# gabrevaya/LatentDiffEq.jl

Measured on NVIDIA B200. Metric: latent trajectory-steps/sec (forward solve + gradient, the reference's ForwardDiffSensitivity semantics), higher is better.
Workload: dtype f32

## Files before the change

### latentdiffeq.jl_b200/csrc/ldeq_api.cu

```cuda
#include <cmath>
#include <cstdio>
#include <cstdlib>
#include <cstring>

#include "ldeq_internal.h"
#include "ldeq_rhs.cuh"
#include "ldeq_tsit5.cuh"
#include "ldeq_julia_trig.cuh"

namespace ldeq {

cudaError_t launch_erk_fwd(int solver, int dtype, bool friction, bool with_tape, const void* z0, const void* theta, const double* tg, int B,
                           int T, const KOpts& ko, void* traj, int32_t* ret, int32_t* na, int32_t* nr, const TapeView<float>& tv,
                           const GridInfo& gi, cudaStream_t s);

int set_err(ldeq_handle* h, int code, const char* what, cudaError_t ce) {
    if (h) {
        h->err = what ? what : "";
        if (ce != cudaSuccess) {
            h->err += ": ";
            h->err += cudaGetErrorString(ce);
        }
    }
    return code;
// ... 152 lines not shown
    if (tape) tv = fwd_tape_view<float>(tape, theta, tg);
    KOpts kov = ko;
    GridInfo giv = gi;
    void* args[] = {&z0, &theta, &tg, &B, &T, &kov, &traj, &ret, &na, &nr, &tv, &giv};
    const int grid = (B + LDEQ_FWD_THREADS - 1) / LDEQ_FWD_THREADS;
    const size_t es = dtype == LDEQ_F32 ? 4 : 8;
    void* kfn = fn[(dtype == LDEQ_F32 ? 0 : 2) + (tape ? 1 : 0)];
    return cudaLaunchKernel(kfn, dim3(grid), dim3(LDEQ_FWD_THREADS), args, ring_smem(rhs->z_dim, es, LDEQ_FWD_THREADS, T), s);
}
static cudaError_t launch_user_bwd(void* const* fn, const ldeq_tape* tape, const void* dtraj, int ld, void* dz0, void* dtheta, cudaStream_t s) {
    TapeView<float> tv{tape->t, (float*)tape->u, tape->info, tape->cap, nullptr, nullptr, nullptr, nullptr, nullptr};
    const void* theta = tape->theta;
    const double* tg = tape->tgrid;
    int B = tape->B, T = tape->T;
    const int32_t* ret = tape->retcode;
    const int32_t* na = tape->naccept;
    GridInfo giv{tape->grid_t0, tape->grid_h, tape->grid_uniform, ld, bwd_sort_lanes()};
    void* args[] = {&theta, &tg, &B, &T, &dtraj, &tv, &ret, &na, &dz0, &dtheta, &giv};
    const int grid = (B + LDEQ_BWD_THREADS - 1) / LDEQ_BWD_THREADS;
    const size_t es = tape->dtype == LDEQ_F32 ? 4 : 8;
    void* kfn = fn[tape->dtype == LDEQ_F32 ? 4 : 5];
    return cudaLaunchKernel(kfn, dim3(grid), dim3(LDEQ_BWD_THREADS), args, ring_smem(tape->z_dim, es, LDEQ_BWD_THREADS, T), s);
}

static cudaError_t launch_user_fwdsens(void* const* fn, const ldeq_tape* tape, const void* dtraj, int ld, void* dz0, void* dtheta, cudaStream_t s) {
    const void* z0 = tape->u;
    const void* theta = tape->theta;
    const double* tg = tape->tgrid;
    int B = tape->B, T = tape->T, np = 1;
    GridInfo gi{tape->grid_t0, tape->grid_h, tape->grid_uniform, ld};
    KOpts kov = tape->kopts;
    const int32_t* ret = tape->retcode;
    const int32_t* key = tape->naccept;
    const int grid = (B + 127) / 128;
    const int base = tape->dtype == LDEQ_F32 ? 6 : 8;
    void* args_p[] = {&z0, &theta, &tg, &B, &gi, &T, &kov, &np, &key, &dtraj, &ret, &dtheta};
    cudaError_t e = cudaLaunchKernel(fn[base], dim3(grid), dim3(128), args_p, 0, s);
    if (e != cudaSuccess) return e;
    void* args_u[] = {&z0, &theta, &tg, &B, &gi, &T, &kov, &np, &key, &dtraj, &ret, &dz0};
    return cudaLaunchKernel(fn[base + 1], dim3(grid), dim3(128), args_u, 0, s);
}

bool slot_acquire(ldeq_handle* h, int32_t** h_info, cudaEvent_t* ev) {
    for (const ldeq_handle::Slot& sl : h->deferred_slots) slot_release(h, sl.h_info, sl.ev);
    h->deferred_slots.clear();
    if (h->free_slots.empty()) {
        const int n = 64;
        int32_t* blk = nullptr;
        if (cudaMallocHost((void**)&blk, n * 2 * sizeof(int32_t)) != cudaSuccess) return false;
        h->pinned_blocks.push_back(blk);
        for (int i = 0; i < n; ++i) {
            cudaEvent_t e;
            if (cudaEventCreateWithFlags(&e, cudaEventDisableTiming) != cudaSuccess) return false;
            h->free_slots.push_back({blk + 2 * i, e});
        }
    }
    ldeq_handle::Slot sl = h->free_slots.back();
    h->free_slots.pop_back();
    *h_info = sl.h_info;
    *ev = sl.ev;
    return true;
}
void slot_release(ldeq_handle* h, int32_t* h_info, cudaEvent_t ev) {
    if (h_info && ev) {
        cudaEventSynchronize(ev);
        if (h) h->free_slots.push_back({h_info, ev});
    }
}
static bool slot_get(ldeq_handle* h, ldeq_tape* tape) { return slot_acquire(h, &tape->h_info, &tape->ready); }
static void slot_put(ldeq_handle* h, ldeq_tape* tape, cudaStream_t s) {
    if (tape->ready && capturing(s))
        h->deferred_slots.push_back({tape->h_info, tape->ready});
    else
// ... 596 lines not shown
```

### latentdiffeq.jl_b200/csrc/ldeq_erk_fwdsens.cu

```cuda
#include "ldeq_fwdsens_kernels.cuh"

namespace ldeq {

template <class MD, class S, bool FR>
static cudaError_t launch_t(const ldeq_tape* tp, const void* dtraj, int ld, void* dz0, void* dtheta, cudaStream_t s) {
    const int B = tp->B, grid = (B + LDEQ_FWDSENS_THREADS - 1) / LDEQ_FWDSENS_THREADS;
    const GridInfo gi{tp->grid_t0, tp->grid_h, tp->grid_uniform, ld};
    const int* key = fwdsens_sort_key(tp);
    erk_fwdsens_kernel<MD, S, 1, FR, true><<<grid, LDEQ_FWDSENS_THREADS, 0, s>>>((const S*)tp->u, (const S*)tp->theta, tp->tgrid, B, gi, tp->T, tp->kopts,
                                                                                1, key, (const S*)dtraj, tp->retcode, (S*)dtheta);
    erk_fwdsens_kernel<MD, S, 2, FR, false><<<grid, LDEQ_FWDSENS_THREADS, 0, s>>>((const S*)tp->u, (const S*)tp->theta, tp->tgrid, B, gi, tp->T, tp->kopts,
                                                                                 1, key, (const S*)dtraj, tp->retcode, (S*)dz0);
    return cudaGetLastError();
}

template <class MD>
static cudaError_t launch_m(const ldeq_tape* tp, const void* dtraj, int ld, void* dz0, void* dtheta, cudaStream_t s) {
    const bool fr = tp->rhs_kind == LDEQ_RHS_PENDULUM_FRICTION;
    if (tp->dtype == LDEQ_F32)
        return fr ? launch_t<MD, float, true>(tp, dtraj, ld, dz0, dtheta, s) : launch_t<MD, float, false>(tp, dtraj, ld, dz0, dtheta, s);
    return fr ? launch_t<MD, double, true>(tp, dtraj, ld, dz0, dtheta, s) : launch_t<MD, double, false>(tp, dtraj, ld, dz0, dtheta, s);
}

cudaError_t launch_erk_fwdsens(const ldeq_tape* tp, const void* dtraj, int ld, void* dz0, void* dtheta, cudaStream_t s) {
    switch (tp->solver) {
        case LDEQ_SOLVER_DP5: return launch_m<ErkDual<TabDP5>>(tp, dtraj, ld, dz0, dtheta, s);
        case LDEQ_SOLVER_BS3: return launch_m<ErkDual<TabBS3>>(tp, dtraj, ld, dz0, dtheta, s);
        case LDEQ_SOLVER_RK4: return launch_m<ErkDual<TabRK4>>(tp, dtraj, ld, dz0, dtheta, s);
        default: return cudaErrorInvalidValue;
    }
}

}
```

### latentdiffeq.jl_b200/csrc/ldeq_fwdsens.cu

```cuda
#include "ldeq_fwdsens_kernels.cuh"

namespace ldeq {

template <class S, bool FR>
static cudaError_t launch_fwdsens_t(const ldeq_tape* tp, const void* dtraj, int ld, void* dz0, void* dtheta, cudaStream_t s) {
    const int B = tp->B, grid = (B + LDEQ_FWDSENS_THREADS - 1) / LDEQ_FWDSENS_THREADS;
    const GridInfo gi{tp->grid_t0, tp->grid_h, tp->grid_uniform, ld};
    const int* key = fwdsens_sort_key(tp);
    tsit5_fwdsens_kernel<S, 1, FR, true><<<grid, LDEQ_FWDSENS_THREADS, 0, s>>>((const S*)tp->u, (const S*)tp->theta, tp->tgrid, B, gi, tp->T, tp->kopts, 1, key,
                                                             (const S*)dtraj, tp->retcode, (S*)dtheta);
    tsit5_fwdsens_kernel<S, 2, FR, false><<<grid, LDEQ_FWDSENS_THREADS, 0, s>>>((const S*)tp->u, (const S*)tp->theta, tp->tgrid, B, gi, tp->T, tp->kopts, 1, key,
                                                              (const S*)dtraj, tp->retcode, (S*)dz0);
    return cudaGetLastError();
}

cudaError_t launch_fwdsens(const ldeq_tape* tp, const void* dtraj, int ld, void* dz0, void* dtheta, cudaStream_t s) {
    if (tp->solver != LDEQ_SOLVER_TSIT5) return launch_erk_fwdsens(tp, dtraj, ld, dz0, dtheta, s);
    const bool fr = tp->rhs_kind == LDEQ_RHS_PENDULUM_FRICTION;
    if (tp->dtype == LDEQ_F32)
        return fr ? launch_fwdsens_t<float, true>(tp, dtraj, ld, dz0, dtheta, s) : launch_fwdsens_t<float, false>(tp, dtraj, ld, dz0, dtheta, s);
    return fr ? launch_fwdsens_t<double, true>(tp, dtraj, ld, dz0, dtheta, s) : launch_fwdsens_t<double, false>(tp, dtraj, ld, dz0, dtheta, s);
}

}
```

### latentdiffeq.jl_b200/csrc/ldeq_fwdsens.cuh

```cuda
#pragma once

#include "ldeq_dual.cuh"
#include "ldeq_erk.cuh"

namespace ldeq {

#define LDEQ_DL _Pragma("unroll") for (int i_ = 0; i_ < N; ++i_)
template <class S, int N> __device__ __forceinline__ Dual<S, N> dual_fma(S s, Dual<S, N> k, Dual<S, N> acc) {
    acc.v = s_fma<S>(s, k.v, acc.v);
    LDEQ_DL acc.d[i_] = s_fma<S>(s, k.d[i_], acc.d[i_]);
    return acc;
}
template <class S, int N> __device__ __forceinline__ Dual<S, N> dual_scale(S a, Dual<S, N> b) {
    b.v *= a;
    LDEQ_DL b.d[i_] *= a;
    return b;
}
template <class S, int N> __device__ __forceinline__ Dual<S, N> dual_axpy_time(Dual<S, N> uprev, double dt, Dual<S, N> sum) {
    Dual<S, N> r;
    r.v = (S)fma(dt, (double)sum.v, (double)uprev.v);
    LDEQ_DL r.d[i_] = (S)fma(dt, (double)sum.d[i_], (double)uprev.d[i_]);
    return r;
}
template <class S, int N> __device__ __forceinline__ Dual<S, N> dual_scale_time(double dt, Dual<S, N> sum) {
    Dual<S, N> r;
    r.v = (S)(dt * (double)sum.v);
    LDEQ_DL r.d[i_] = (S)(dt * (double)sum.d[i_]);
    return r;
}
template <class S, int N> __device__ __forceinline__ S dual_sse(Dual<S, N> a, bool wp) {
    S s = a.v * a.v;
    if (wp) { LDEQ_DL s += a.d[i_] * a.d[i_]; }
    return s;
}
template <class S, int N> __device__ __forceinline__ S dual_absnorm(Dual<S, N> a, bool wp) { return wp ? s_sqrt<S>(dual_sse(a, true)) : s_abs<S>(a.v); }
template <class S, int N> __device__ __forceinline__ Dual<S, N> dual_div_s(Dual<S, N> a, S s) {
    a.v /= s;
    LDEQ_DL a.d[i_] /= s;
    return a;
}
template <class S, int N> __device__ __forceinline__ S dual_rms(const Dual<S, N>* a, int n, bool wp) {
    S s = (S)0;
    for (int i = 0; i < n; ++i) s += dual_sse(a[i], wp);
    const int len = wp ? n * (1 + N) : n;
    return s_sqrt<S>(s / (S)len);
}
#undef LDEQ_DL

#ifndef LDEQ_FWDSENS_PREFETCH_ROWS
#define LDEQ_FWDSENS_PREFETCH_ROWS 24
#endif
#ifndef LDEQ_FWDSENS_THREADS
#define LDEQ_FWDSENS_THREADS 128
#endif

__device__ __forceinline__ void prefetch_l1(const void* p) { asm volatile("prefetch.global.L1 [%0];" ::"l"(p)); }

struct Tsit5Dual {
    static constexpr int NS = 7, ORDER = 5;
    template <class RHS, class S, int NP>
    __device__ __forceinline__ static void step(const Dual<S, NP>* u, const Dual<S, NP>* L, double t, double dts,
                                                Dual<S, NP> (*k)[RHS::ZD], Dual<S, NP>* unew) {
        constexpr int Z = RHS::ZD;
        using D = Dual<S, NP>;
        using Tb = Tab<S>;
        D tmp[Z], sum;
        for (int i = 0; i < Z; ++i) { sum = dual_scale(Tb::a21, k[0][i]); tmp[i] = dual_axpy_time(u[i], dts, sum); }
        RHS::f(k[1], tmp, L, t + Tb::c2 * dts);
        for (int i = 0; i < Z; ++i) {
            sum = dual_scale(Tb::a31, k[0][i]); sum = dual_fma(Tb::a32, k[1][i], sum);
            tmp[i] = dual_axpy_time(u[i], dts, sum);
        }
        RHS::f(k[2], tmp, L, t + Tb::c3 * dts);
        for (int i = 0; i < Z; ++i) {
            sum = dual_scale(Tb::a41, k[0][i]); sum = dual_fma(Tb::a42, k[1][i], sum); sum = dual_fma(Tb::a43, k[2][i], sum);
            tmp[i] = dual_axpy_time(u[i], dts, sum);
        }
        RHS::f(k[3], tmp, L, t + Tb::c4 * dts);
        for (int i = 0; i < Z; ++i) {
            sum = dual_scale(Tb::a51, k[0][i]); sum = dual_fma(Tb::a52, k[1][i], sum); sum = dual_fma(Tb::a53, k[2][i], sum);
            sum = dual_fma(Tb::a54, k[3][i], sum);
            tmp[i] = dual_axpy_time(u[i], dts, sum);
        }
        RHS::f(k[4], tmp, L, t + Tb::c5 * dts);
        for (int i = 0; i < Z; ++i) {
            sum = dual_scale(Tb::a61, k[0][i]); sum = dual_fma(Tb::a62, k[1][i], sum); sum = dual_fma(Tb::a63, k[2][i], sum);
            sum = dual_fma(Tb::a64, k[3][i], sum); sum = dual_fma(Tb::a65, k[4][i], sum);
            tmp[i] = dual_axpy_time(u[i], dts, sum);
        }
        RHS::f(k[5], tmp, L, t + dts);
        for (int i = 0; i < Z; ++i) {
            sum = dual_scale(Tb::a71, k[0][i]); sum = dual_fma(Tb::a72, k[1][i], sum); sum = dual_fma(Tb::a73, k[2][i], sum);
            sum = dual_fma(Tb::a74, k[3][i], sum); sum = dual_fma(Tb::a75, k[4][i], sum); sum = dual_fma(Tb::a76, k[5][i], sum);
            unew[i] = dual_axpy_time(u[i], dts, sum);
        }
        RHS::f(k[6], unew, L, t + dts);
    }
    template <class S, int NP, int Z>
    __device__ __forceinline__ static Dual<S, NP> err_sum(Dual<S, NP> (*k)[Z], int i) {
        using Tb = Tab<S>;
        Dual<S, NP> sum = dual_scale(Tb::bt1, k[0][i]);
        sum = dual_fma(Tb::bt2, k[1][i], sum); sum = dual_fma(Tb::bt3, k[2][i], sum);
        sum = dual_fma(Tb::bt4, k[3][i], sum); sum = dual_fma(Tb::bt5, k[4][i], sum); sum = dual_fma(Tb::bt6, k[5][i], sum);
        sum = dual_fma(Tb::bt7, k[6][i], sum);
        return sum;
    }
    __device__ __forceinline__ static void dense_c(const double* kk, double* c2, double* c3, double* c4) {
        using Td = Tab<double>;
        *c2 = fma(Td::r72, kk[6], fma(Td::r62, kk[5], fma(Td::r52, kk[4], fma(Td::r42, kk[3], fma(Td::r32, kk[2], fma(Td::r22, kk[1], Td::r12 * kk[0]))))));
        *c3 = fma(Td::r73, kk[6], fma(Td::r63, kk[5], fma(Td::r53, kk[4], fma(Td::r43, kk[3], fma(Td::r33, kk[2], fma(Td::r23, kk[1], Td::r13 * kk[0]))))));
        *c4 = fma(Td::r74, kk[6], fma(Td::r64, kk[5], fma(Td::r54, kk[4], fma(Td::r44, kk[3], fma(Td::r34, kk[2], fma(Td::r24, kk[1], Td::r14 * kk[0]))))));
    }
};

template <class TB> struct ErkDual {
    static constexpr int NS = TB::NS, ORDER = TB::ORDER;
    template <class RHS, class S, int NP>
    __device__ __forceinline__ static void step(const Dual<S, NP>* u, const Dual<S, NP>* L, double t, double dts,
                                                Dual<S, NP> (*k)[RHS::ZD], Dual<S, NP>* unew) {
        constexpr int Z = RHS::ZD;
        using D = Dual<S, NP>;
        D tmp[Z];
#pragma unroll
        for (int j = 1; j < NS; ++j) {
            for (int i = 0; i < Z; ++i) {
                D sum = D((S)0);
                bool first = true;
#pragma unroll
                for (int l = 0; l < j; ++l) {
                    if (TB::a(j, l) == 0.0) continue;
                    sum = first ? dual_scale((S)TB::a(j, l), k[l][i]) : dual_fma((S)TB::a(j, l), k[l][i], sum);
                    first = false;
                }
                if (j < NS - 1) tmp[i] = dual_axpy_time(u[i], dts, sum);
                else unew[i] = dual_axpy_time(u[i], dts, sum);
            }
            if (j < NS - 1) RHS::f(k[j], tmp, L, t + TB::c(j) * dts);
            else RHS::f(k[j], unew, L, t + dts);
        }
    }
    template <class S, int NP, int Z>
    __device__ __forceinline__ static Dual<S, NP> err_sum(Dual<S, NP> (*k)[Z], int i) {
        Dual<S, NP> sum = Dual<S, NP>((S)0);
        bool first = true;
#pragma unroll
        for (int j = 0; j < NS; ++j) {
            if (TB::bt(j) == 0.0) continue;
            sum = first ? dual_scale((S)TB::bt(j), k[j][i]) : dual_fma((S)TB::bt(j), k[j][i], sum);
            first = false;
        }
        return sum;
    }
    __device__ __forceinline__ static void dense_c(const double* kk, double* c2, double* c3, double* c4) {
        double c[3] = {0.0, 0.0, 0.0};
#pragma unroll
        for (int m = 1; m < 4; ++m)
#pragma unroll
            for (int j = 0; j < NS; ++j)
                if (erk_r<TB>(j, m) != 0.0) c[m - 1] = fma(erk_r<TB>(j, m), kk[j], c[m - 1]);
        *c2 = c[0]; *c3 = c[1]; *c4 = c[2];
    }
};

template <class M, class RHS, class S, int NP, bool SEED_P>
__device__ __forceinline__ void
erk_fwdsens_body(const S* __restrict__ z0, const S* __restrict__ theta, const double* __restrict__ tg, int B, GridInfo gi, int T,
                   KOpts o, int norm_partials, const int* __restrict__ sort_key, const S* __restrict__ dtraj, const int* __restrict__ primal_ret,
                   S* __restrict__ dout) {
    constexpr int Z = RHS::ZD, PD = RHS::PD;
    using D = Dual<S, NP>;
    constexpr int NS = M::NS;
    int b = blockIdx.x * blockDim.x + threadIdx.x;
    const int ld = gi.ld;
    auto tgrid = [&](int k) -> double { return gi.uniform ? fma((double)k, gi.h, gi.t0) : tg[k]; };
    const bool wp = norm_partials != 0;
    if (sort_key) {
        __shared__ int s_key[LDEQ_FWDSENS_THREADS];
        __shared__ short s_order[LDEQ_FWDSENS_THREADS];
        const int tid = threadIdx.x, nt = blockDim.x;
        const int key = b < B ? sort_key[b] : 0x7fffffff;
        s_key[tid] = key;
        __syncthreads();
        int rank = 0;
        for (int j = 0; j < nt; ++j) {
            const int kj = s_key[j];
            rank += (kj < key || (kj == key && j < tid)) ? 1 : 0;
        }
        s_order[rank] = (short)tid;
        __syncthreads();
        b = blockIdx.x * blockDim.x + s_order[tid];
    }
    if (b >= B) return;
    D u[Z], k[NS][Z], unew[Z], tmp[Z], sum, L[PD + RHS::NPRE];
    const double t0 = tg[0], tend = tg[T - 1];
    const double dtmax = o.dtmax > 0.0 ? o.dtmax : (tend - t0);
    const double dtmin = o.dtmin > 0.0 ? o.dtmin : fmax(2.220446049250313e-16, ulp_of(t0));
    const S abstol = (S)o.abstol, reltol = (S)o.reltol;
    double acc[NP];
    double t = t0, dt = o.dt;
    {
        {
            for (int i = 0; i < Z; ++i) {
                u[i] = D(z0[(size_t)b * Z + i]);
                if (!SEED_P) u[i].d[i] = (S)1;
            }
            for (int i = 0; i < PD; ++i) {
                L[i] = D(theta[(size_t)b * PD + i]);
                if (SEED_P) L[i].d[i] = (S)1;
            }
            RHS::prepare(L);
            RHS::f(k[0], u, L, t0);
            if (o.adaptive && !(o.dt > 0.0)) {
                S sk[Z];
                for (int i = 0; i < Z; ++i) {
                    sk[i] = abstol + dual_absnorm(u[i], wp) * reltol;
                    tmp[i] = dual_div_s(u[i], sk[i]);
                }
                const double d0 = (double)dual_rms(tmp, Z, wp);
                for (int i = 0; i < Z; ++i) tmp[i] = dual_div_s(k[0][i], sk[i]);
                const double d1 = (double)dual_rms(tmp, Z, wp);
                double dt0 = (d0 < 1e-5 || d1 < 1e-5) ? 1e-6 : 0.01 * (d0 / d1);
                dt0 = fmin(dt0, dtmax);
                if (dt0 < 10.0 * 2.220446049250313e-16) {
                    dt = fmax(1e-6, dtmin);
                } else {
                    D u1[Z], f1[Z];
                    for (int i = 0; i < Z; ++i) u1[i] = dual_axpy_time(u[i], dt0, k[0][i]);
                    RHS::f(f1, u1, L, t0 + dt0);
                    for (int i = 0; i < Z; ++i) tmp[i] = dual_div_s(f1[i] - k[0][i], sk[i]);
                    const double d2 = (double)dual_rms(tmp, Z, wp) / dt0;
                    const double m = fmax(d1, d2);
                    const double dt1 = (m <= 1e-15) ? fmax(1e-6, dt0 * 1e-3) : ::pow(10.0, -(2.0 + log10(m)) / (double)M::ORDER);
                    dt = fmax(dtmin, fmin(100.0 * dt0, fmin(dt1, dtmax)));
                }
            }
        }
    }
#pragma unroll
    for (int q = 0; q < NP; ++q) acc[q] = 0.0;
    for (int i = 0; i < Z; ++i)
#pragma unroll
        for (int q = 0; q < NP; ++q) acc[q] += (double)u[i].d[q] * (double)dtraj[(size_t)b * Z + i];
    PiState pst = pi_init(o);
    int ks = 1, ret = RET_SUCCESS;
    long long iters = 0;
    if (!(dt > 0.0) || !isfinite(dt)) ret = RET_DTLESSTHANMIN;
    int kpf = 1;
    S dvn[Z];
#pragma unroll
    for (int i = 0; i < Z; ++i) dvn[i] = T > 1 ? dtraj[((size_t)ld + b) * Z + i] : (S)0;
    while (ks < T && ret == RET_SUCCESS) {
        if (iters >= o.maxiters) { ret = RET_MAXITERS; break; }
        ++iters;
        {
            const int hi = ks + LDEQ_FWDSENS_PREFETCH_ROWS < T ? ks + LDEQ_FWDSENS_PREFETCH_ROWS : T;
            for (; kpf < hi; ++kpf) prefetch_l1(dtraj + ((size_t)kpf * ld + b) * Z);
        }
        const double dts = fmin(dt, tend - t);
        double tnew = t + dts;
        if (::fabs(tnew - tend) < 100.0 * ulp_of(fmax(::fabs(t), ::fabs(tend)))) tnew = tend;
        M::template step<RHS, S, NP>(u, L, t, dts, k, unew);
        double EEst = 0.0;
// ... 26 lines not shown
                for (int i = 0; i < Z; ++i) dv[i] = dvn[i];
                if (ks + 1 < T) {
#pragma unroll
                    for (int i = 0; i < Z; ++i) dvn[i] = dtraj[((size_t)(ks + 1) * ld + b) * Z + i];
                }
                if (tsv == tnew) {
#pragma unroll
                    for (int i = 0; i < Z; ++i)
#pragma unroll
                        for (int q = 0; q < NP; ++q) acc[q] += (double)unew[i].d[q] * (double)dv[i];
                } else {
                    const S th = (S)((tsv - t) * inv);
                    const S a1 = (S)dts * th, a2 = a1 * th, a3 = a2 * th, a4 = a3 * th;
#pragma unroll
                    for (int i = 0; i < Z; ++i) {
                        wsum[i] += dv[i];
                        w1[i] = s_fma<S>(a1, dv[i], w1[i]);
                        w2[i] = s_fma<S>(a2, dv[i], w2[i]);
                        w3[i] = s_fma<S>(a3, dv[i], w3[i]);
                        w4[i] = s_fma<S>(a4, dv[i], w4[i]);
                    }
                    interior = true;
                }
                ++ks;
                tsv = ks < T ? tgrid(ks) : 0.0;
            }
            if (interior) {
#pragma unroll
                for (int i = 0; i < Z; ++i)
#pragma unroll
                    for (int q = 0; q < NP; ++q) {
                        double kk[NS], c2, c3, c4;
#pragma unroll
                        for (int j = 0; j < NS; ++j) kk[j] = (double)k[j][i].d[q];
                        const double k1 = kk[0];
                        M::dense_c(kk, &c2, &c3, &c4);
                        acc[q] += (double)u[i].d[q] * (double)wsum[i] +
                                  (k1 * (double)w1[i] + c2 * (double)w2[i] + c3 * (double)w3[i] + c4 * (double)w4[i]);
                    }
            }
            t = tnew;
            for (int i = 0; i < Z; ++i) { u[i] = unew[i]; k[0][i] = k[NS - 1][i]; }
        }
        if (o.adaptive) dt = dt_next;
        if (ks < T && o.adaptive && (!(::fabs(dt) > dtmin) || !isfinite(dt))) { ret = RET_DTLESSTHANMIN; break; }
    }
    const bool ok = ret == RET_SUCCESS && primal_ret[b] == RET_SUCCESS;
#pragma unroll
    for (int q = 0; q < NP; ++q) dout[(size_t)b * NP + q] = ok ? (S)acc[q] : (S)0;
}

template <class RHS, class S, int NP, bool SEED_P>
__device__ __forceinline__ void
tsit5_fwdsens_body(const S* __restrict__ z0, const S* __restrict__ theta, const double* __restrict__ tg, int B, GridInfo gi, int T,
                   KOpts o, int norm_partials, const int* __restrict__ sort_key, const S* __restrict__ dtraj, const int* __restrict__ primal_ret,
                   S* __restrict__ dout) {
    erk_fwdsens_body<Tsit5Dual, RHS, S, NP, SEED_P>(z0, theta, tg, B, gi, T, o, norm_partials, sort_key, dtraj, primal_ret, dout);
}

}
```

### latentdiffeq.jl_b200/csrc/ldeq_fwdsens_kernels.cuh

```cuda
#pragma once
#include "ldeq_internal.h"
#include "ldeq_fwdsens.cuh"
#include <cstdlib>

#ifndef LDEQ_FWDSENS_MINBLOCKS
#define LDEQ_FWDSENS_MINBLOCKS 5
#endif

namespace ldeq {

template <bool FRICTION> struct PendulumDualRHS {
    static constexpr int ZD = 2, PD = 1;
    static constexpr int NPRE = 1;
    template <class D> __device__ __forceinline__ static void prepare(D* p) {
        typedef typename D::value_type S;
        const D G((S)10.0f);
        p[PD] = -G / p[0];
    }
    template <class D> __device__ __forceinline__ static void f(D* du, const D* u, const D* p, double) {
        typedef typename D::value_type S;
        du[0] = u[1];
        const D a = p[PD] * sin(u[0]);
        if (FRICTION) {
            const S bm = (S)0.7f / (S)1.0f;
            du[1] = a - bm * u[1];
        } else {
            du[1] = a;
        }
    }
};

template <class S, int NP, bool FRICTION, bool SEED_P>
__global__ void __launch_bounds__(LDEQ_FWDSENS_THREADS, LDEQ_FWDSENS_MINBLOCKS)
tsit5_fwdsens_kernel(const S* __restrict__ z0, const S* __restrict__ theta, const double* __restrict__ tg, int B, GridInfo gi, int T,
                     KOpts o, int norm_partials, const int* __restrict__ sort_key, const S* __restrict__ dtraj, const int* __restrict__ primal_ret,
                     S* __restrict__ dout) {
    tsit5_fwdsens_body<PendulumDualRHS<FRICTION>, S, NP, SEED_P>(z0, theta, tg, B, gi, T, o, norm_partials, sort_key, dtraj, primal_ret, dout);
}

template <class MD, class S, int NP, bool FRICTION, bool SEED_P>
__global__ void __launch_bounds__(LDEQ_FWDSENS_THREADS, LDEQ_FWDSENS_MINBLOCKS)
erk_fwdsens_kernel(const S* __restrict__ z0, const S* __restrict__ theta, const double* __restrict__ tg, int B, GridInfo gi, int T,
                   KOpts o, int norm_partials, const int* __restrict__ sort_key, const S* __restrict__ dtraj, const int* __restrict__ primal_ret,
                   S* __restrict__ dout) {
    erk_fwdsens_body<MD, PendulumDualRHS<FRICTION>, S, NP, SEED_P>(z0, theta, tg, B, gi, T, o, norm_partials, sort_key, dtraj, primal_ret, dout);
}

inline const int* fwdsens_sort_key(const ldeq_tape* tp) {
    static const bool sort = [] { const char* e = getenv("LDEQ_FWDSENS_SORT"); return !(e && e[0] == '0'); }();
    return sort ? tp->naccept : nullptr;
}

}
```

### latentdiffeq.jl_b200/csrc/ldeq_internal.h

```cpp
#pragma once

#include <cuda_runtime.h>
#include <stdint.h>

#include <string>
#include <vector>

#include "../../include/ldeq.h"
#include "ldeq_common.cuh"

#define LDEQ_MAX_SLABS 8
#define LDEQ_GRID_CACHE 16

struct ldeq_handle {
    int device = 0;
    std::string err;
    int64_t launches = 0;
    double* d_tgrid = nullptr;
    size_t d_tgrid_cap = 0;
    std::vector<double> h_tgrid;
    double grid_t0 = 0.0, grid_h = 0.0;
    int grid_uniform = 0;
    struct GridEntry {
        std::vector<double> t;
// ... 41 lines not shown
    const ldeq_rhs* rhs = nullptr;
    void* base = nullptr;
    double* t = nullptr;
    void* u = nullptr;
    void* theta = nullptr;
    double* tgrid = nullptr;
    int32_t* retcode = nullptr;
    int32_t* naccept = nullptr;
    int32_t* nreject = nullptr;
    int32_t* info = nullptr;
    int32_t* h_info = nullptr;
    cudaEvent_t ready = nullptr;
    bool checked = false;
    ldeq::KOpts kopts;
    double grid_t0 = 0.0, grid_h = 0.0;
    int grid_uniform = 0;
    int sense = 0;
    int solver = 0;
    std::vector<ldeq_tape*> parts;
    std::vector<int> part_b0;
};

namespace ldeq {

int set_err(ldeq_handle* h, int code, const char* what, cudaError_t ce = cudaSuccess);
bool capturing(cudaStream_t s);
int refuse_capture(ldeq_handle* h, cudaStream_t s, const char* what, const char* why);
int upload_tgrid(ldeq_handle* h, const double* t_host, int T, cudaStream_t s);
int ensure_scratch(ldeq_handle* h, int slot, size_t bytes, cudaStream_t s);
KOpts to_kopts(const ldeq_opts* o);
int bwd_sort_lanes();
bool slot_acquire(ldeq_handle* h, int32_t** h_info, cudaEvent_t* ev);
void slot_release(ldeq_handle* h, int32_t* h_info, cudaEvent_t ev);
cudaError_t launch_fwdsens(const ldeq_tape* tape, const void* dtraj, int ld, void* dz0, void* dtheta, cudaStream_t s);
cudaError_t launch_erk_fwdsens(const ldeq_tape* tape, const void* dtraj, int ld, void* dz0, void* dtheta, cudaStream_t s);
cudaError_t launch_erk_bwd(const ldeq_tape* tape, const void* dtraj, int ld, void* dz0, void* dtheta, cudaStream_t s);
void* const* user_rhs_kernels(ldeq_handle* h, const ldeq_rhs* rhs, int solver);

#define LDEQ_CUDA(call)                                                    \
    do {                                                                   \
        cudaError_t _e = (call);                                           \
        if (_e != cudaSuccess) return ldeq::set_err(h, LDEQ_ERR_CUDA, #call, _e); \
    } while (0)

}
```

### latentdiffeq.jl_b200/csrc/ldeq_user_rhs.cu

```cuda
#include <dlfcn.h>

#include <cstdio>
#include <string>
#include <vector>

#include "ldeq_internal.h"

namespace {
#include "ldeq_embedded.inc"

typedef struct _nvrtcProgram* nvrtcProgram;
struct Nvrtc {
    void* lib = nullptr;
    int (*CreateProgram)(nvrtcProgram*, const char*, const char*, int, const char* const*, const char* const*) = nullptr;
    int (*CompileProgram)(nvrtcProgram, int, const char* const*) = nullptr;
    int (*GetCUBINSize)(nvrtcProgram, size_t*) = nullptr;
    int (*GetCUBIN)(nvrtcProgram, char*) = nullptr;
    int (*GetProgramLogSize)(nvrtcProgram, size_t*) = nullptr;
    int (*GetProgramLog)(nvrtcProgram, char*) = nullptr;
    int (*DestroyProgram)(nvrtcProgram*) = nullptr;
    const char* (*GetErrorString)(int) = nullptr;
};

Nvrtc* nvrtc() {
// ... 10 lines not shown
    LDEQ_SYM(CreateProgram) LDEQ_SYM(CompileProgram) LDEQ_SYM(GetCUBINSize) LDEQ_SYM(GetCUBIN)
    LDEQ_SYM(GetProgramLogSize) LDEQ_SYM(GetProgramLog) LDEQ_SYM(DestroyProgram) LDEQ_SYM(GetErrorString)
#undef LDEQ_SYM
    return &n;
}

const char* kWrapper = R"LDEQ(
using namespace ldeq;
#define LDEQ_USER_FWD(NAME, S, TAPE)                                                                              \
    extern "C" __global__ void __launch_bounds__(LDEQ_FWD_THREADS, LDEQ_FWD_MINBLOCKS)                             \
    NAME(const S* __restrict__ z0, const S* __restrict__ theta, const double* __restrict__ tg, int B, int T, KOpts o, \
         S* __restrict__ traj, int* __restrict__ retcode, int* __restrict__ naccept, int* __restrict__ nreject,    \
         TapeView<S> tape, GridInfo ginfo) {                                                                      \
        erk_fwd_body<LDEQ_USER_M, UserRHS<S, LDEQ_USER_ZD, LDEQ_USER_PD>, S, TAPE>(z0, theta, tg, B, T, o, traj,   \
                                                                        retcode, naccept, nreject, tape, ginfo);  \
    }
#define LDEQ_USER_BWD(NAME, S)                                                                                    \
    extern "C" __global__ void __launch_bounds__(LDEQ_BWD_THREADS, LDEQ_BWD_MINBLOCKS)                             \
    NAME(const S* __restrict__ theta, const double* __restrict__ tg, int B, int T, const S* __restrict__ dtraj,   \
         TapeView<S> tape, const int* __restrict__ retcode, const int* __restrict__ naccept, S* __restrict__ dz0, \
         S* __restrict__ dtheta, GridInfo ginfo) {                                                                \
        erk_bwd_body<LDEQ_USER_M, UserRHS<S, LDEQ_USER_ZD, LDEQ_USER_PD>, S>(theta, tg, B, T, dtraj, tape, retcode, \
                                                                  naccept, dz0, dtheta, ginfo);                   \
    }
// LDEQ_SENSE_FORWARD_DUAL: the reference's dual-number re-solves with the user's function (ldeq_fwdsens.cuh)
struct UserDualRHS {
    static constexpr int ZD = LDEQ_USER_ZD, PD = LDEQ_USER_PD, NPRE = 0;
    template <class D> __device__ __forceinline__ static void prepare(D*) {}
    template <class D> __device__ __forceinline__ static void f(D* du, const D* u, const D* p, double t) {
        ::ldeq_user_rhs<D>(du, u, p, D((typename D::value_type)t));
    }
};
#define LDEQ_USER_FWDSENS(NAME, S, SEED_P)                                                                        \
    extern "C" __global__ void __launch_bounds__(128)                                                             \
    NAME(const S* __restrict__ z0, const S* __restrict__ theta, const double* __restrict__ tg, int B, GridInfo gi, int T, KOpts o, \
         int norm_partials, const int* __restrict__ sort_key, const S* __restrict__ dtraj,                          \
         const int* __restrict__ primal_ret, S* __restrict__ dout) {                                                \
        erk_fwdsens_body<LDEQ_USER_MD, UserDualRHS, S, (SEED_P ? LDEQ_USER_PD : LDEQ_USER_ZD), SEED_P>(           \
            z0, theta, tg, B, gi, T, o, norm_partials, sort_key, dtraj, primal_ret, dout);                                    \
    }
LDEQ_USER_FWD(ldeq_user_fwd_f32, float, false)
LDEQ_USER_FWD(ldeq_user_fwd_f32_tape, float, true)
LDEQ_USER_FWD(ldeq_user_fwd_f64, double, false)
LDEQ_USER_FWD(ldeq_user_fwd_f64_tape, double, true)
LDEQ_USER_BWD(ldeq_user_bwd_f32, float)
LDEQ_USER_BWD(ldeq_user_bwd_f64, double)
LDEQ_USER_FWDSENS(ldeq_user_fwdsens_p_f32, float, true)
LDEQ_USER_FWDSENS(ldeq_user_fwdsens_u_f32, float, false)
LDEQ_USER_FWDSENS(ldeq_user_fwdsens_p_f64, double, true)
LDEQ_USER_FWDSENS(ldeq_user_fwdsens_u_f64, double, false)
)LDEQ";

const int kNumKernels = 10;
const char* kKernelNames[kNumKernels] = {"ldeq_user_fwd_f32", "ldeq_user_fwd_f32_tape", "ldeq_user_fwd_f64",
                                         "ldeq_user_fwd_f64_tape", "ldeq_user_bwd_f32", "ldeq_user_bwd_f64",
                                         "ldeq_user_fwdsens_p_f32", "ldeq_user_fwdsens_u_f32",
                                         "ldeq_user_fwdsens_p_f64", "ldeq_user_fwdsens_u_f64"};
}

using namespace ldeq;

namespace {

const char* kMethodDefs[4] = {
    "#define LDEQ_USER_M Tsit5M\n#define LDEQ_USER_MD Tsit5Dual\n",
    "#define LDEQ_USER_M DP5M\n#define LDEQ_USER_MD ErkDual<TabDP5>\n",
    "#define LDEQ_USER_M BS3M\n#define LDEQ_USER_MD ErkDual<TabBS3>\n",
    "#define LDEQ_USER_M RK4M\n#define LDEQ_USER_MD ErkDual<TabRK4>\n",
};

int compile_variant(ldeq_handle* h, const char* cuda_src, int z_dim, int p_dim, int solver, void** module_out, void** fn_out) {
    Nvrtc* n = nvrtc();
    if (!n) return set_err(h, LDEQ_ERR_COMPILE, "libnvrtc.so.12 could not be loaded (needed for user-defined right-hand sides)");
    LDEQ_CUDA(cudaSetDevice(h->device));
    std::string src;
    src += "#define LDEQ_USER_ZD " + std::to_string(z_dim) + "\n#define LDEQ_USER_PD " + std::to_string(p_dim) + "\n";
    src += kMethodDefs[solver];
    src += ldeq_src_common;
    src += ldeq_src_erk;
    src += ldeq_src_tsit5;
    src += ldeq_src_jltrig;
    src += ldeq_src_dual;
    src += ldeq_src_fwdsens;
    src += "\n// ---- user source ----\n";
    src += cuda_src;
    src += "\n";
    src += kWrapper;
    nvrtcProgram prog = nullptr;
    int rc = n->CreateProgram(&prog, src.c_str(), "ldeq_user_rhs.cu", 0, nullptr, nullptr);
    if (rc) return set_err(h, LDEQ_ERR_COMPILE, n->GetErrorString(rc));
    const char* opts[] = {"--gpu-architecture=sm_100a", "--std=c++17", "-default-device", "--fmad=true",
                          "-DLDEQ_NVRTC=1", "-lineinfo"};
    rc = n->CompileProgram(prog, 6, opts);
    if (rc) {
        size_t ls = 0;
        n->GetProgramLogSize(prog, &ls);
        std::string log(ls, '\0');
        if (ls) n->GetProgramLog(prog, &log[0]);
        n->DestroyProgram(&prog);
        h->err = std::string("NVRTC: ") + n->GetErrorString(rc) + "\n" + log;
        return LDEQ_ERR_COMPILE;
    }
    size_t cs = 0;
    n->GetCUBINSize(prog, &cs);
    std::vector<char> cubin(cs);
    n->GetCUBIN(prog, cubin.data());
    n->DestroyProgram(&prog);
    cudaLibrary_t lib = nullptr;
    cudaError_t e = cudaLibraryLoadData(&lib, cubin.data(), nullptr, nullptr, 0, nullptr, nullptr, 0);
    if (e != cudaSuccess) return set_err(h, LDEQ_ERR_CUDA, "cudaLibraryLoadData(user rhs cubin)", e);
    for (int i = 0; i < kNumKernels; ++i) {
        cudaKernel_t k = nullptr;
        e = cudaLibraryGetKernel(&k, lib, kKernelNames[i]);
        if (e != cudaSuccess) {
            cudaLibraryUnload(lib);
            return set_err(h, LDEQ_ERR_CUDA, "cudaLibraryGetKernel(user rhs)", e);
        }
        fn_out[i] = (void*)k;
    }
    *module_out = (void*)lib;
    return LDEQ_OK;
}

}

namespace ldeq {

void* const* user_rhs_kernels(ldeq_handle* h, const ldeq_rhs* rhs, int solver) {
    if (solver == LDEQ_SOLVER_TSIT5) return rhs->fn;
    if (solver < 0 || solver > LDEQ_SOLVER_RK4) { set_err(h, LDEQ_ERR_UNSUPPORTED, "solver"); return nullptr; }
    ldeq_rhs* r = const_cast<ldeq_rhs*>(rhs);
    if (!r->alt[solver].module) {
        void* mod = nullptr;
        if (compile_variant(h, r->user_src.c_str(), r->z_dim, r->p_dim, solver, &mod, r->alt[solver].fn) != LDEQ_OK) return nullptr;
        r->alt[solver].module = mod;
    }
    return r->alt[solver].fn;
}

}

extern "C" {

int ldeq_rhs_from_source(ldeq_handle* h, const char* cuda_src, int z_dim, int p_dim, ldeq_rhs** out) {
    if (!h || !out) return LDEQ_ERR_INVALID;
    *out = nullptr;
    if (!cuda_src) return set_err(h, LDEQ_ERR_INVALID, "null source");
    if (z_dim < 1 || z_dim > 8 || p_dim < 1 || p_dim > 8)
        return set_err(h, LDEQ_ERR_UNSUPPORTED, "user rhs: 1 <= z_dim <= 8 and 1 <= p_dim <= 8 (state lives in registers)");
    ldeq_rhs* r = new ldeq_rhs();
    r->kind = -1;
    r->z_dim = z_dim;
// ... 19 lines not shown
```

Measured before the change: 29.33 billion.

## Move forward-dual RK stage buffers into shared memory to cut register pressure

Stores the Runge-Kutta stage derivatives (dual numbers) in a per-thread strided shared-memory slab instead of a register/local array, sized per solver, state and parameter dimension. The f32 minimum-blocks launch bound rises from 5 to 8, and user kernels get thread counts and dynamic smem limits picked to fit. The aim is to avoid local-memory spills and raise occupancy. The cost is shared-memory traffic on every stage access, including volatile accesses that block register caching, plus an extra barrier.

```diff
diff --git a/latentdiffeq.jl_b200/csrc/ldeq_api.cu b/latentdiffeq.jl_b200/csrc/ldeq_api.cu
--- a/latentdiffeq.jl_b200/csrc/ldeq_api.cu
+++ b/latentdiffeq.jl_b200/csrc/ldeq_api.cu
@@ -208,13 +208,17 @@
     KOpts kov = tape->kopts;
     const int32_t* ret = tape->retcode;
     const int32_t* key = tape->naccept;
-    const int grid = (B + 127) / 128;
+    const int threads = user_fwdsens_threads(tape->z_dim, tape->p_dim), grid = (B + threads - 1) / threads;
     const int base = tape->dtype == LDEQ_F32 ? 6 : 8;
+    const size_t es = tape->dtype == LDEQ_F32 ? 4 : 8;
+    const int ns = erk_stages(tape->solver);
     void* args_p[] = {&z0, &theta, &tg, &B, &gi, &T, &kov, &np, &key, &dtraj, &ret, &dtheta};
-    cudaError_t e = cudaLaunchKernel(fn[base], dim3(grid), dim3(128), args_p, 0, s);
+    cudaError_t e = cudaLaunchKernel(fn[base], dim3(grid), dim3(threads), args_p,
+                                     fwdsens_smem_bytes(ns, tape->z_dim, tape->p_dim, es, threads), s);
     if (e != cudaSuccess) return e;
     void* args_u[] = {&z0, &theta, &tg, &B, &gi, &T, &kov, &np, &key, &dtraj, &ret, &dz0};
-    return cudaLaunchKernel(fn[base + 1], dim3(grid), dim3(128), args_u, 0, s);
+    return cudaLaunchKernel(fn[base + 1], dim3(grid), dim3(threads), args_u,
+                            fwdsens_smem_bytes(ns, tape->z_dim, tape->z_dim, es, threads), s);
 }
 
 bool slot_acquire(ldeq_handle* h, int32_t** h_info, cudaEvent_t* ev) {
diff --git a/latentdiffeq.jl_b200/csrc/ldeq_erk_fwdsens.cu b/latentdiffeq.jl_b200/csrc/ldeq_erk_fwdsens.cu
--- a/latentdiffeq.jl_b200/csrc/ldeq_erk_fwdsens.cu
+++ b/latentdiffeq.jl_b200/csrc/ldeq_erk_fwdsens.cu
@@ -1,15 +1,19 @@
 #include "ldeq_fwdsens_kernels.cuh"
 
 namespace ldeq {
+
+static_assert(erk_stages(LDEQ_SOLVER_TSIT5) == Tsit5Dual::NS && erk_stages(LDEQ_SOLVER_DP5) == TabDP5::NS &&
+                  erk_stages(LDEQ_SOLVER_BS3) == TabBS3::NS && erk_stages(LDEQ_SOLVER_RK4) == TabRK4::NS,
+              "erk_stages (host sizing of the user forward-dual slab) out of step with the method tables");
 
 template <class MD, class S, bool FR>
 static cudaError_t launch_t(const ldeq_tape* tp, const void* dtraj, int ld, void* dz0, void* dtheta, cudaStream_t s) {
     const int B = tp->B, grid = (B + LDEQ_FWDSENS_THREADS - 1) / LDEQ_FWDSENS_THREADS;
     const GridInfo gi{tp->grid_t0, tp->grid_h, tp->grid_uniform, ld};
     const int* key = fwdsens_sort_key(tp);
-    erk_fwdsens_kernel<MD, S, 1, FR, true><<<grid, LDEQ_FWDSENS_THREADS, 0, s>>>((const S*)tp->u, (const S*)tp->theta, tp->tgrid, B, gi, tp->T, tp->kopts,
+    erk_fwdsens_kernel<MD, S, 1, FR, true><<<grid, LDEQ_FWDSENS_THREADS, pendulum_fwdsens_smem<MD, S, 1>(), s>>>((const S*)tp->u, (const S*)tp->theta, tp->tgrid, B, gi, tp->T, tp->kopts,
                                                                                 1, key, (const S*)dtraj, tp->retcode, (S*)dtheta);
-    erk_fwdsens_kernel<MD, S, 2, FR, false><<<grid, LDEQ_FWDSENS_THREADS, 0, s>>>((const S*)tp->u, (const S*)tp->theta, tp->tgrid, B, gi, tp->T, tp->kopts,
+    erk_fwdsens_kernel<MD, S, 2, FR, false><<<grid, LDEQ_FWDSENS_THREADS, pendulum_fwdsens_smem<MD, S, 2>(), s>>>((const S*)tp->u, (const S*)tp->theta, tp->tgrid, B, gi, tp->T, tp->kopts,
                                                                                  1, key, (const S*)dtraj, tp->retcode, (S*)dz0);
     return cudaGetLastError();
 }
diff --git a/latentdiffeq.jl_b200/csrc/ldeq_fwdsens.cu b/latentdiffeq.jl_b200/csrc/ldeq_fwdsens.cu
--- a/latentdiffeq.jl_b200/csrc/ldeq_fwdsens.cu
+++ b/latentdiffeq.jl_b200/csrc/ldeq_fwdsens.cu
@@ -7,9 +7,9 @@
     const int B = tp->B, grid = (B + LDEQ_FWDSENS_THREADS - 1) / LDEQ_FWDSENS_THREADS;
     const GridInfo gi{tp->grid_t0, tp->grid_h, tp->grid_uniform, ld};
     const int* key = fwdsens_sort_key(tp);
-    tsit5_fwdsens_kernel<S, 1, FR, true><<<grid, LDEQ_FWDSENS_THREADS, 0, s>>>((const S*)tp->u, (const S*)tp->theta, tp->tgrid, B, gi, tp->T, tp->kopts, 1, key,
+    tsit5_fwdsens_kernel<S, 1, FR, true><<<grid, LDEQ_FWDSENS_THREADS, pendulum_fwdsens_smem<Tsit5Dual, S, 1>(), s>>>((const S*)tp->u, (const S*)tp->theta, tp->tgrid, B, gi, tp->T, tp->kopts, 1, key,
                                                              (const S*)dtraj, tp->retcode, (S*)dtheta);
-    tsit5_fwdsens_kernel<S, 2, FR, false><<<grid, LDEQ_FWDSENS_THREADS, 0, s>>>((const S*)tp->u, (const S*)tp->theta, tp->tgrid, B, gi, tp->T, tp->kopts, 1, key,
+    tsit5_fwdsens_kernel<S, 2, FR, false><<<grid, LDEQ_FWDSENS_THREADS, pendulum_fwdsens_smem<Tsit5Dual, S, 2>(), s>>>((const S*)tp->u, (const S*)tp->theta, tp->tgrid, B, gi, tp->T, tp->kopts, 1, key,
                                                               (const S*)dtraj, tp->retcode, (S*)dz0);
     return cudaGetLastError();
 }
diff --git a/latentdiffeq.jl_b200/csrc/ldeq_fwdsens.cuh b/latentdiffeq.jl_b200/csrc/ldeq_fwdsens.cuh
--- a/latentdiffeq.jl_b200/csrc/ldeq_fwdsens.cuh
+++ b/latentdiffeq.jl_b200/csrc/ldeq_fwdsens.cuh
@@ -56,53 +56,83 @@
 
 __device__ __forceinline__ void prefetch_l1(const void* p) { asm volatile("prefetch.global.L1 [%0];" ::"l"(p)); }
 
+template <class S, int NP, int Z> struct DualStages {
+    static constexpr int NT = LDEQ_FWDSENS_THREADS;
+    volatile S* p;
+    __device__ __forceinline__ Dual<S, NP> operator()(int j, int i) const {
+        const volatile S* q = p + (j * Z + i) * (NP + 1) * NT;
+        Dual<S, NP> r;
+        r.v = q[0];
+#pragma unroll
+        for (int m = 0; m < NP; ++m) r.d[m] = q[(m + 1) * NT];
+        return r;
+    }
+    __device__ __forceinline__ S partial(int j, int i, int m) const { return p[((j * Z + i) * (NP + 1) + 1 + m) * NT]; }
+    __device__ __forceinline__ void set(int j, int i, const Dual<S, NP>& x) const {
+        volatile S* q = p + (j * Z + i) * (NP + 1) * NT;
+        q[0] = x.v;
+#pragma unroll
+        for (int m = 0; m < NP; ++m) q[(m + 1) * NT] = x.d[m];
+    }
+    __device__ __forceinline__ void set(int j, const Dual<S, NP>* x) const {
+#pragma unroll
+        for (int i = 0; i < Z; ++i) set(j, i, x[i]);
+    }
+};
+
 struct Tsit5Dual {
     static constexpr int NS = 7, ORDER = 5;
     template <class RHS, class S, int NP>
     __device__ __forceinline__ static void step(const Dual<S, NP>* u, const Dual<S, NP>* L, double t, double dts,
-                                                Dual<S, NP> (*k)[RHS::ZD], Dual<S, NP>* unew) {
+                                                const DualStages<S, NP, RHS::ZD>& k, Dual<S, NP>* unew) {
         constexpr int Z = RHS::ZD;
         using D = Dual<S, NP>;
         using Tb = Tab<S>;
-        D tmp[Z], sum;
-        for (int i = 0; i < Z; ++i) { sum = dual_scale(Tb::a21, k[0][i]); tmp[i] = dual_axpy_time(u[i], dts, sum); }
-        RHS::f(k[1], tmp, L, t + Tb::c2 * dts);
-        for (int i = 0; i < Z; ++i) {
-            sum = dual_scale(Tb::a31, k[0][i]); sum = dual_fma(Tb::a32, k[1][i], sum);
+        D tmp[Z], kj[Z], sum;
+        for (int i = 0; i < Z; ++i) { sum = dual_scale(Tb::a21, k(0, i)); tmp[i] = dual_axpy_time(u[i], dts, sum); }
+        RHS::f(kj, tmp, L, t + Tb::c2 * dts);
+        k.set(1, kj);
+        for (int i = 0; i < Z; ++i) {
+            sum = dual_scale(Tb::a31, k(0, i)); sum = dual_fma(Tb::a32, k(1, i), sum);
             tmp[i] = dual_axpy_time(u[i], dts, sum);
         }
-        RHS::f(k[2], tmp, L, t + Tb::c3 * dts);
-        for (int i = 0; i < Z; ++i) {
-            sum = dual_scale(Tb::a41, k[0][i]); sum = dual_fma(Tb::a42, k[1][i], sum); sum = dual_fma(Tb::a43, k[2][i], sum);
+        RHS::f(kj, tmp, L, t + Tb::c3 * dts);
+        k.set(2, kj);
+        for (int i = 0; i < Z; ++i) {
+            sum = dual_scale(Tb::a41, k(0, i)); sum = dual_fma(Tb::a42, k(1, i), sum); sum = dual_fma(Tb::a43, k(2, i), sum);
             tmp[i] = dual_axpy_time(u[i], dts, sum);
         }
-        RHS::f(k[3], tmp, L, t + Tb::c4 * dts);
-        for (int i = 0; i < Z; ++i) {
-            sum = dual_scale(Tb::a51, k[0][i]); sum = dual_fma(Tb::a52, k[1][i], sum); sum = dual_fma(Tb::a53, k[2][i], sum);
-            sum = dual_fma(Tb::a54, k[3][i], sum);
+        RHS::f(kj, tmp, L, t + Tb::c4 * dts);
+        k.set(3, kj);
+        for (int i = 0; i < Z; ++i) {
+            sum = dual_scale(Tb::a51, k(0, i)); sum = dual_fma(Tb::a52, k(1, i), sum); sum = dual_fma(Tb::a53, k(2, i), sum);
+            sum = dual_fma(Tb::a54, k(3, i), sum);
             tmp[i] = dual_axpy_time(u[i], dts, sum);
         }
-        RHS::f(k[4], tmp, L, t + Tb::c5 * dts);
-        for (int i = 0; i < Z; ++i) {
-            sum = dual_scale(Tb::a61, k[0][i]); sum = dual_fma(Tb::a62, k[1][i], sum); sum = dual_fma(Tb::a63, k[2][i], sum);
-            sum = dual_fma(Tb::a64, k[3][i], sum); sum = dual_fma(Tb::a65, k[4][i], sum);
+        RHS::f(kj, tmp, L, t + Tb::c5 * dts);
+        k.set(4, kj);
+        for (int i = 0; i < Z; ++i) {
+            sum = dual_scale(Tb::a61, k(0, i)); sum = dual_fma(Tb::a62, k(1, i), sum); sum = dual_fma(Tb::a63, k(2, i), sum);
+            sum = dual_fma(Tb::a64, k(3, i), sum); sum = dual_fma(Tb::a65, k(4, i), sum);
             tmp[i] = dual_axpy_time(u[i], dts, sum);
         }
-        RHS::f(k[5], tmp, L, t + dts);
-        for (int i = 0; i < Z; ++i) {
-            sum = dual_scale(Tb::a71, k[0][i]); sum = dual_fma(Tb::a72, k[1][i], sum); sum = dual_fma(Tb::a73, k[2][i], sum);
-            sum = dual_fma(Tb::a74, k[3][i], sum); sum = dual_fma(Tb::a75, k[4][i], sum); sum = dual_fma(Tb::a76, k[5][i], sum);
+        RHS::f(kj, tmp, L, t + dts);
+        k.set(5, kj);
+        for (int i = 0; i < Z; ++i) {
+            sum = dual_scale(Tb::a71, k(0, i)); sum = dual_fma(Tb::a72, k(1, i), sum); sum = dual_fma(Tb::a73, k(2, i), sum);
+            sum = dual_fma(Tb::a74, k(3, i), sum); sum = dual_fma(Tb::a75, k(4, i), sum); sum = dual_fma(Tb::a76, k(5, i), sum);
             unew[i] = dual_axpy_time(u[i], dts, sum);
         }
-        RHS::f(k[6], unew, L, t + dts);
+        RHS::f(kj, unew, L, t + dts);
+        k.set(6, kj);
     }
     template <class S, int NP, int Z>
-    __device__ __forceinline__ static Dual<S, NP> err_sum(Dual<S, NP> (*k)[Z], int i) {
+    __device__ __forceinline__ static Dual<S, NP> err_sum(const DualStages<S, NP, Z>& k, int i) {
         using Tb = Tab<S>;
-        Dual<S, NP> sum = dual_scale(Tb::bt1, k[0][i]);
-        sum = dual_fma(Tb::bt2, k[1][i], sum); sum = dual_fma(Tb::bt3, k[2][i], sum);
-        sum = dual_fma(Tb::bt4, k[3][i], sum); sum = dual_fma(Tb::bt5, k[4][i], sum); sum = dual_fma(Tb::bt6, k[5][i], sum);
-        sum = dual_fma(Tb::bt7, k[6][i], sum);
+        Dual<S, NP> sum = dual_scale(Tb::bt1, k(0, i));
+        sum = dual_fma(Tb::bt2, k(1, i), sum); sum = dual_fma(Tb::bt3, k(2, i), sum);
+        sum = dual_fma(Tb::bt4, k(3, i), sum); sum = dual_fma(Tb::bt5, k(4, i), sum); sum = dual_fma(Tb::bt6, k(5, i), sum);
+        sum = dual_fma(Tb::bt7, k(6, i), sum);
         return sum;
     }
     __device__ __forceinline__ static void dense_c(const double* kk, double* c2, double* c3, double* c4) {
@@ -117,10 +147,10 @@
     static constexpr int NS = TB::NS, ORDER = TB::ORDER;
     template <class RHS, class S, int NP>
     __device__ __forceinline__ static void step(const Dual<S, NP>* u, const Dual<S, NP>* L, double t, double dts,
-                                                Dual<S, NP> (*k)[RHS::ZD], Dual<S, NP>* unew) {
+                                                const DualStages<S, NP, RHS::ZD>& k, Dual<S, NP>* unew) {
         constexpr int Z = RHS::ZD;
         using D = Dual<S, NP>;
-        D tmp[Z];
+        D tmp[Z], kj[Z];
 #pragma unroll
         for (int j = 1; j < NS; ++j) {
             for (int i = 0; i < Z; ++i) {
@@ -129,24 +159,25 @@
 #pragma unroll
                 for (int l = 0; l < j; ++l) {
                     if (TB::a(j, l) == 0.0) continue;
-                    sum = first ? dual_scale((S)TB::a(j, l), k[l][i]) : dual_fma((S)TB::a(j, l), k[l][i], sum);
+                    sum = first ? dual_scale((S)TB::a(j, l), k(l, i)) : dual_fma((S)TB::a(j, l), k(l, i), sum);
                     first = false;
                 }
                 if (j < NS - 1) tmp[i] = dual_axpy_time(u[i], dts, sum);
                 else unew[i] = dual_axpy_time(u[i], dts, sum);
             }
-            if (j < NS - 1) RHS::f(k[j], tmp, L, t + TB::c(j) * dts);
-            else RHS::f(k[j], unew, L, t + dts);
+            if (j < NS - 1) RHS::f(kj, tmp, L, t + TB::c(j) * dts);
+            else RHS::f(kj, unew, L, t + dts);
+            k.set(j, kj);
         }
     }
     template <class S, int NP, int Z>
-    __device__ __forceinline__ static Dual<S, NP> err_sum(Dual<S, NP> (*k)[Z], int i) {
+    __device__ __forceinline__ static Dual<S, NP> err_sum(const DualStages<S, NP, Z>& k, int i) {
         Dual<S, NP> sum = Dual<S, NP>((S)0);
         bool first = true;
 #pragma unroll
         for (int j = 0; j < NS; ++j) {
             if (TB::bt(j) == 0.0) continue;
-            sum = first ? dual_scale((S)TB::bt(j), k[j][i]) : dual_fma((S)TB::bt(j), k[j][i], sum);
+            sum = first ? dual_scale((S)TB::bt(j), k(j, i)) : dual_fma((S)TB::bt(j), k(j, i), sum);
             first = false;
         }
         return sum;
@@ -174,9 +205,10 @@
     const int ld = gi.ld;
     auto tgrid = [&](int k) -> double { return gi.uniform ? fma((double)k, gi.h, gi.t0) : tg[k]; };
     const bool wp = norm_partials != 0;
+    extern __shared__ __align__(16) unsigned char fwdsens_smem[];
     if (sort_key) {
-        __shared__ int s_key[LDEQ_FWDSENS_THREADS];
-        __shared__ short s_order[LDEQ_FWDSENS_THREADS];
+        int* s_key = reinterpret_cast<int*>(fwdsens_smem);
+        short* s_order = reinterpret_cast<short*>(s_key + LDEQ_FWDSENS_THREADS);
         const int tid = threadIdx.x, nt = blockDim.x;
         const int key = b < B ? sort_key[b] : 0x7fffffff;
         s_key[tid] = key;
@@ -189,9 +221,11 @@
         s_order[rank] = (short)tid;
         __syncthreads();
         b = blockIdx.x * blockDim.x + s_order[tid];
+        __syncthreads();
     }
     if (b >= B) return;
-    D u[Z], k[NS][Z], unew[Z], tmp[Z], sum, L[PD + RHS::NPRE];
+    const DualStages<S, NP, Z> k{reinterpret_cast<S*>(fwdsens_smem) + threadIdx.x};
+    D u[Z], unew[Z], tmp[Z], sum, L[PD + RHS::NPRE];
     const double t0 = tg[0], tend = tg[T - 1];
     const double dtmax = o.dtmax > 0.0 ? o.dtmax : (tend - t0);
     const double dtmin = o.dtmin > 0.0 ? o.dtmin : fmax(2.220446049250313e-16, ulp_of(t0));
@@ -209,7 +243,8 @@
                 if (SEED_P) L[i].d[i] = (S)1;
             }
             RHS::prepare(L);
-            RHS::f(k[0], u, L, t0);
+            RHS::f(tmp, u, L, t0);
+            k.set(0, tmp);
             if (o.adaptive && !(o.dt > 0.0)) {
                 S sk[Z];
                 for (int i = 0; i < Z; ++i) {
@@ -217,7 +252,7 @@
                     tmp[i] = dual_div_s(u[i], sk[i]);
                 }
                 const double d0 = (double)dual_rms(tmp, Z, wp);
-                for (int i = 0; i < Z; ++i) tmp[i] = dual_div_s(k[0][i], sk[i]);
+                for (int i = 0; i < Z; ++i) tmp[i] = dual_div_s(k(0, i), sk[i]);
                 const double d1 = (double)dual_rms(tmp, Z, wp);
                 double dt0 = (d0 < 1e-5 || d1 < 1e-5) ? 1e-6 : 0.01 * (d0 / d1);
                 dt0 = fmin(dt0, dtmax);
@@ -225,9 +260,9 @@
                     dt = fmax(1e-6, dtmin);
                 } else {
                     D u1[Z], f1[Z];
-                    for (int i = 0; i < Z; ++i) u1[i] = dual_axpy_time(u[i], dt0, k[0][i]);
+                    for (int i = 0; i < Z; ++i) u1[i] = dual_axpy_time(u[i], dt0, k(0, i));
                     RHS::f(f1, u1, L, t0 + dt0);
-                    for (int i = 0; i < Z; ++i) tmp[i] = dual_div_s(f1[i] - k[0][i], sk[i]);
+                    for (int i = 0; i < Z; ++i) tmp[i] = dual_div_s(f1[i] - k(0, i), sk[i]);
                     const double d2 = (double)dual_rms(tmp, Z, wp) / dt0;
                     const double m = fmax(d1, d2);
                     const double dt1 = (m <= 1e-15) ? fmax(1e-6, dt0 * 1e-3) : ::pow(10.0, -(2.0 + log10(m)) / (double)M::ORDER);
@@ -320,7 +355,7 @@
                     for (int q = 0; q < NP; ++q) {
                         double kk[NS], c2, c3, c4;
 #pragma unroll
-                        for (int j = 0; j < NS; ++j) kk[j] = (double)k[j][i].d[q];
+                        for (int j = 0; j < NS; ++j) kk[j] = (double)k.partial(j, i, q);
                         const double k1 = kk[0];
                         M::dense_c(kk, &c2, &c3, &c4);
                         acc[q] += (double)u[i].d[q] * (double)wsum[i] +
@@ -328,7 +363,7 @@
                     }
             }
             t = tnew;
-            for (int i = 0; i < Z; ++i) { u[i] = unew[i]; k[0][i] = k[NS - 1][i]; }
+            for (int i = 0; i < Z; ++i) { u[i] = unew[i]; k.set(0, i, k(NS - 1, i)); }
         }
         if (o.adaptive) dt = dt_next;
         if (ks < T && o.adaptive && (!(::fabs(dt) > dtmin) || !isfinite(dt))) { ret = RET_DTLESSTHANMIN; break; }
diff --git a/latentdiffeq.jl_b200/csrc/ldeq_fwdsens_kernels.cuh b/latentdiffeq.jl_b200/csrc/ldeq_fwdsens_kernels.cuh
--- a/latentdiffeq.jl_b200/csrc/ldeq_fwdsens_kernels.cuh
+++ b/latentdiffeq.jl_b200/csrc/ldeq_fwdsens_kernels.cuh
@@ -4,8 +4,12 @@
 #include <cstdlib>
 
 #ifndef LDEQ_FWDSENS_MINBLOCKS
-#define LDEQ_FWDSENS_MINBLOCKS 5
+#define LDEQ_FWDSENS_MINBLOCKS 8
 #endif
+#ifndef LDEQ_FWDSENS_MINBLOCKS_F64
+#define LDEQ_FWDSENS_MINBLOCKS_F64 5
+#endif
+#define LDEQ_FWDSENS_BOUNDS(S) __launch_bounds__(LDEQ_FWDSENS_THREADS, sizeof(S) == 4 ? LDEQ_FWDSENS_MINBLOCKS : LDEQ_FWDSENS_MINBLOCKS_F64)
 
 namespace ldeq {
 
@@ -31,7 +35,7 @@
 };
 
 template <class S, int NP, bool FRICTION, bool SEED_P>
-__global__ void __launch_bounds__(LDEQ_FWDSENS_THREADS, LDEQ_FWDSENS_MINBLOCKS)
+__global__ void LDEQ_FWDSENS_BOUNDS(S)
 tsit5_fwdsens_kernel(const S* __restrict__ z0, const S* __restrict__ theta, const double* __restrict__ tg, int B, GridInfo gi, int T,
                      KOpts o, int norm_partials, const int* __restrict__ sort_key, const S* __restrict__ dtraj, const int* __restrict__ primal_ret,
                      S* __restrict__ dout) {
@@ -39,11 +43,17 @@
 }
 
 template <class MD, class S, int NP, bool FRICTION, bool SEED_P>
-__global__ void __launch_bounds__(LDEQ_FWDSENS_THREADS, LDEQ_FWDSENS_MINBLOCKS)
+__global__ void LDEQ_FWDSENS_BOUNDS(S)
 erk_fwdsens_kernel(const S* __restrict__ z0, const S* __restrict__ theta, const double* __restrict__ tg, int B, GridInfo gi, int T,
                    KOpts o, int norm_partials, const int* __restrict__ sort_key, const S* __restrict__ dtraj, const int* __restrict__ primal_ret,
                    S* __restrict__ dout) {
     erk_fwdsens_body<MD, PendulumDualRHS<FRICTION>, S, NP, SEED_P>(z0, theta, tg, B, gi, T, o, norm_partials, sort_key, dtraj, primal_ret, dout);
+}
+
+template <class M, class S, int NP> constexpr size_t pendulum_fwdsens_smem() {
+    constexpr size_t bytes = fwdsens_smem_bytes(M::NS, 2, NP, sizeof(S), LDEQ_FWDSENS_THREADS);
+    static_assert(bytes <= 48 * 1024, "stage slab above the default dynamic shared memory limit");
+    return bytes;
 }
 
 inline const int* fwdsens_sort_key(const ldeq_tape* tp) {
diff --git a/latentdiffeq.jl_b200/csrc/ldeq_internal.h b/latentdiffeq.jl_b200/csrc/ldeq_internal.h
--- a/latentdiffeq.jl_b200/csrc/ldeq_internal.h
+++ b/latentdiffeq.jl_b200/csrc/ldeq_internal.h
@@ -97,6 +97,14 @@
 int bwd_sort_lanes();
 bool slot_acquire(ldeq_handle* h, int32_t** h_info, cudaEvent_t* ev);
 void slot_release(ldeq_handle* h, int32_t* h_info, cudaEvent_t ev);
+constexpr size_t fwdsens_smem_bytes(int ns, int z, int np, size_t es, int threads) { return (size_t)ns * z * (np + 1) * es * threads; }
+constexpr int erk_stages(int solver) { return solver == LDEQ_SOLVER_BS3 ? 4 : solver == LDEQ_SOLVER_RK4 ? 5 : 7; }
+inline int user_fwdsens_threads(int z_dim, int p_dim) {
+    const int np = z_dim > p_dim ? z_dim : p_dim;
+    int threads = 128;
+    while (threads > 32 && fwdsens_smem_bytes(7, z_dim, np, 8, threads) > 227 * 1024) threads /= 2;
+    return threads;
+}
 cudaError_t launch_fwdsens(const ldeq_tape* tape, const void* dtraj, int ld, void* dz0, void* dtheta, cudaStream_t s);
 cudaError_t launch_erk_fwdsens(const ldeq_tape* tape, const void* dtraj, int ld, void* dz0, void* dtheta, cudaStream_t s);
 cudaError_t launch_erk_bwd(const ldeq_tape* tape, const void* dtraj, int ld, void* dz0, void* dtheta, cudaStream_t s);
diff --git a/latentdiffeq.jl_b200/csrc/ldeq_user_rhs.cu b/latentdiffeq.jl_b200/csrc/ldeq_user_rhs.cu
--- a/latentdiffeq.jl_b200/csrc/ldeq_user_rhs.cu
+++ b/latentdiffeq.jl_b200/csrc/ldeq_user_rhs.cu
@@ -66,7 +66,7 @@
     }
 };
 #define LDEQ_USER_FWDSENS(NAME, S, SEED_P)                                                                        \
-    extern "C" __global__ void __launch_bounds__(128)                                                             \
+    extern "C" __global__ void __launch_bounds__(LDEQ_FWDSENS_THREADS)                                            \
     NAME(const S* __restrict__ z0, const S* __restrict__ theta, const double* __restrict__ tg, int B, GridInfo gi, int T, KOpts o, \
          int norm_partials, const int* __restrict__ sort_key, const S* __restrict__ dtraj,                          \
          const int* __restrict__ primal_ret, S* __restrict__ dout) {                                                \
@@ -109,6 +109,7 @@
     LDEQ_CUDA(cudaSetDevice(h->device));
     std::string src;
     src += "#define LDEQ_USER_ZD " + std::to_string(z_dim) + "\n#define LDEQ_USER_PD " + std::to_string(p_dim) + "\n";
+    src += "#define LDEQ_FWDSENS_THREADS " + std::to_string(user_fwdsens_threads(z_dim, p_dim)) + "\n";
     src += kMethodDefs[solver];
     src += ldeq_src_common;
     src += ldeq_src_erk;
@@ -152,6 +153,18 @@
         }
         fn_out[i] = (void*)k;
     }
+    const int threads = user_fwdsens_threads(z_dim, p_dim), ns = erk_stages(solver);
+    for (int i = 6; i < 10; ++i) {
+        const size_t es = i < 8 ? 4 : 8;
+        const int np = (i % 2 == 0) ? p_dim : z_dim;
+        const size_t bytes = fwdsens_smem_bytes(ns, z_dim, np, es, threads);
+        if (bytes <= 48 * 1024) continue;
+        e = cudaFuncSetAttribute(fn_out[i], cudaFuncAttributeMaxDynamicSharedMemorySize, (int)bytes);
+        if (e != cudaSuccess) {
+            cudaLibraryUnload(lib);
+            return set_err(h, LDEQ_ERR_CUDA, "cudaFuncSetAttribute(user rhs forward-dual kernel)", e);
+        }
+    }
     *module_out = (void*)lib;
     return LDEQ_OK;
 }
```

New measurement: 28.95 billion, median of 6. -1.3%, worse.
